# dmalyuta/explicit_hybrid_mpc

Hardware: AMD Instinct MI355X
Metric: oracle LP solves/sec + final regions/sec, 4-state 2-input N=5 hybrid MPC (higher is better)
Workload: dtype f64

## Files before the change

explicit_hybrid_mpc_amd/csrc/ehm_capi.hip:

```cpp
#include <hip/hip_runtime.h>

#include <algorithm>
#include <cmath>
#include <cstdarg>
#include <cstdio>
#include <cstdlib>
#include <cstring>
#include <functional>
#include <memory>
#include <set>
#include <string>
#include <vector>

#include "../../include/ehmpc.h"
#include "ehm_host.h"
#include "ehm_batch_host.h"

#define EHM_MAX_P_DEV 8
#include "ehm_kernels.h"
#include "ehm_k2.h"
#include "ehm_implicit.h"

using namespace ehm;

// ... 367 lines not shown
        const int id = nodes[t / (p + 1)];
        const int v = t % (p + 1);
        double* rec = T.rec + (size_t)id * T.rec_stride;
        if (lane < p) th[lane] = rec[v * p + lane];
        wave_sync();
        LpWork w;
        double b[EHM_SLOTS];
        assemble_point(w, lp_base, P, T.didx[id], th, false, b, lane);
        const IpmResult r = ipm_solve(w, b, lane);
        count_solve(cnt, r, lane);
        if (r.status != 0 && lane == 0) atomicAdd(&cnt->errors, 1ULL);
        if (lane == 0) rec[rec_off_vcost(p) + v] = r.obj;
        if (lane < n_u) rec[rec_off_vinput(p) + v * n_u + lane] = w.xb[lane];
    }
}

static thread_local ehm_err_channel g_err;

#define HIP_TRY(expr, code)                                                              \
    do {                                                                                 \
        hipError_t e_ = (expr);                                                          \
        if (e_ != hipSuccess)                                                            \
            return g_err.fail(code, "%s failed: %s (%s:%d)", #expr,                      \
                              hipGetErrorString(e_), __FILE__, __LINE__);                \
    } while (0)

struct NodePool {
    long long cap = 0;
    DevBuf rec, left, didx, depth, flags, tstar, grad, wit, mt_state, mt_data;
};

struct ehm_problem {
    int device = 0;
    Stream stream;
    DevProblem dp{};
    int delta_len = 0;
    std::vector<uint8_t> deltas;
    DevBuf consts;
    DevBuf wc2;
    DevBuf wc4;
    DevBuf wr3;
    DevBuf quad;
    bool quadratic = false;
    bool k2q_ok = false;
    bool v1_ok = false;
    int decide_full = 0;
    int mid_first = 1;
    int inherit_wit = 1;
    bool budget_keep = false;
    bool check_witness = false;
    int work_first = 1;
    int eager_children = 1;
    int requeue_undecided = 1;
    int share_mid = 1;
    int any_admissible = 0;
    int hy_timing = 0;
    int solver_gen = 2;
    DevBuf seg;
    std::set<const K2Api*> k2_ready;
    std::set<const KpApi*> kp_ready;
    NodePool pool_cache;
    DevBuf fr_a, fr_b, open_flag, open_list, d_count;
    DevBuf pq_slots, pq_ctl;
    DevBuf in0, in1, in2, out0, out1, out2, out3;
    DevBuf ex_stage, ex_tmp;
    DevBuf d_cnt;
    DevCounters* counters() const { return d_cnt.as<DevCounters>(); }
    struct ehm_tree* active_run = nullptr;
    std::vector<struct ehm_tree*> trees;
    Event bev[2];
    double batch_seconds[2] = {0.0, 0.0};
    long long batch_launches[2] = {0, 0};
    long long launches = 0;
    long long fallbacks = 0;
    long long slivers = 0;
    int num_cu = 256;
    size_t lds_point = 0, lds_simplex = 0, lds_expand = 0;
};

struct HyState;

struct ehm_tree {
    ehm_problem* prob = nullptr;
    int device = 0;
    std::unique_ptr<HyState> hy;
    DevTree dt{};
    NodePool pool;
    long long limit = 0;
    DevBuf code;
    ehm_tree_info info{};
    int skip_volume = 0;
    int32_t persist_kernel[4] = {0, 0, 0, 0};
    bool unordered = false;
    bool keep_ids = false;
    DevBuf d_perm, d_inv;
    bool have_perm = false;
    struct Run {
        bool active = false;
        int max_depth = 0, action = 0, shard_world = 1, shard_rank = 0, engine = 0;
        int deal_depth = 0;
        long long shard_min = 0;
        bool sharded = true, cur_is_a = true;
        long long n_roots = 0, n_nodes = 0, nf = 0, n_closed = 0, ref_solves = 0;
        long long pre_closed = 0, pre_nodes = 0, pre_solves = 0, given = 0, received = 0;
        long long pre_first = 0;
        long long pushes = 0;
        int sweeps = 0, depth = 0, truncated = 0;
        DevCounters c0{};
        Event ev0;
        std::vector<Event> evs;
        std::vector<int> ev_kind;
    } run;
    ~ehm_tree();
};

static int map_deltas(ehm_problem* P, int64_t n_inst, const uint8_t* delta,
                      std::vector<int32_t>& out) {
    out.resize((size_t)n_inst);
    const int L = P->delta_len;
    for (int64_t k = 0; k < n_inst; ++k) {
// ... 496 lines not shown
        return g_err.fail(EHM_E_NO_DEVICE, "no HIP device %d (libehmpc has no CPU fallback)",
                          device);
    HIP_TRY(hipSetDevice(device), EHM_E_NO_DEVICE);
    DevBuf d_out;
    HIP_TRY(d_out.alloc(5 * sizeof(double)), EHM_E_HIP);
    int k = 0;
    for (k2_getter g : g_k2_getters) {
        if (k >= max_instances) break;
        g()->selftest(nullptr, d_out.as<double>());
        HIP_TRY(hipDeviceSynchronize(), EHM_E_HIP);
        HIP_TRY(hipMemcpy(out + 5 * k, d_out.ptr, 5 * sizeof(double), hipMemcpyDeviceToHost),
                EHM_E_HIP);
        ++k;
    }
    *n_instances = k;
    return EHM_OK;
}

int ehm_problem_set_option(ehm_problem* P, const char* name, double value) {
    if (!P || !name) return g_err.fail(EHM_E_INVALID, "null argument");
    if (!strcmp(name, "solver")) return ehm_problem_set_solver(P, (int)value);
    if (!strcmp(name, "decide_full")) {
        P->decide_full = value != 0.0;
        return EHM_OK;
    }
    if (!strcmp(name, "timing")) {
        P->hy_timing = value != 0.0;
        return EHM_OK;
    }
    if (!strcmp(name, "mid_first")) {
        P->mid_first = value != 0.0;
        return EHM_OK;
    }
    if (!strcmp(name, "inherit_witness")) {
        P->inherit_wit = value != 0.0;
        return EHM_OK;
    }
    if (!strcmp(name, "work_first")) {
        P->work_first = value != 0.0;
        return EHM_OK;
    }
    if (!strcmp(name, "check_witness")) {
        P->check_witness = value != 0.0;
        return EHM_OK;
    }
    if (!strcmp(name, "eager_children")) {
        P->eager_children = value != 0.0;
        return EHM_OK;
    }
    if (!strcmp(name, "requeue_undecided")) {
        P->requeue_undecided = value != 0.0;
        return EHM_OK;
    }
    if (!strcmp(name, "budget_keep")) {
        P->budget_keep = value != 0.0;
        return EHM_OK;
    }
    if (!strcmp(name, "share_midpoints")) {
        P->share_mid = value != 0.0;
        return EHM_OK;
    }
    if (!strcmp(name, "any_admissible")) {
        if (value < 0.0 || value > 2e9)
            return g_err.fail(EHM_E_INVALID, "any_admissible: seed + 1, or 0");
        if (P->active_run)
            return g_err.fail(EHM_E_INVALID, "any_admissible: not while a partition run is active");
        P->any_admissible = (int)value;
        return EHM_OK;
    }
    return g_err.fail(EHM_E_INVALID, "unknown option '%s'", name);
}

int ehm_sync(ehm_problem* P) {
    if (!P) return g_err.fail(EHM_E_INVALID, "null problem");
    HIP_TRY(hipStreamSynchronize(P->stream), EHM_E_HIP);
    return EHM_OK;
}

void* ehm_stream(ehm_problem* P) { return P ? (void*)P->stream : nullptr; }

int ehm_stats(ehm_problem* P, ehm_counters* out) {
    if (!P || !out) return g_err.fail(EHM_E_INVALID, "null argument");
    HIP_TRY(hipSetDevice(P->device), EHM_E_HIP);
    DevCounters c;
    HIP_TRY(hipStreamSynchronize(P->stream), EHM_E_HIP);
    HIP_TRY(hipMemcpy(&c, P->counters(), sizeof c, hipMemcpyDeviceToHost), EHM_E_HIP);
    out->lp_solves = (int64_t)c.lp_solves;
    out->ipm_iters = (int64_t)c.ipm_iters;
    out->stalled = (int64_t)c.stalled;
    out->kernel_launches = P->launches;
    out->fallbacks = P->fallbacks;
    out->slivers = P->slivers;
    for (int k = 0; k < 2; ++k) {
        out->batch_seconds[k] = P->batch_seconds[k];
        out->batch_launches[k] = P->batch_launches[k];
    }
    return EHM_OK;
}

struct BatchIn {
    const double* host;
    size_t width;
    DevBuf* dev;
};
struct BatchOut {
    void* host;
// ... 1190 lines not shown
        }
    }
    const long long waves = (long long)cfg.L.grid * (cfg.L.threads / 64);
    const long long n_slots = 2 * T->limit + waves + 64;
    if (n_slots > 0x7fffffffLL || T->limit >= (long long)EHM_REQUEUED)
        return g_err.fail(EHM_E_INVALID, "node pool too large for the persistent engine");
    HIP_TRY(P->pq_slots.ensure((size_t)n_slots * 4), EHM_E_HIP);
    HIP_TRY(P->pq_ctl.ensure(sizeof(PersistCtl)), EHM_E_HIP);
    int32_t* slots = P->pq_slots.as<int32_t>();
    HIP_TRY(hipMemsetAsync(slots, 0xFF, (size_t)n_slots * 4, P->stream), EHM_E_HIP);
    const int32_t* cur = (R.cur_is_a ? P->fr_a : P->fr_b).as<int32_t>();
    HIP_TRY(hipMemcpyAsync(slots, cur, (size_t)R.nf * 4, hipMemcpyDeviceToDevice, P->stream),
            EHM_E_HIP);
    PersistDeal deal{0, 0, 0, 1, 0, 0, 0, 0};
    deal.check = P->check_witness ? 1 : 0;
    T->dt.code = nullptr;
    if (dealt) {
        deal = PersistDeal{0, R.deal_depth, R.shard_rank, R.shard_world,
                           getenv("EHM_DEAL_LOW_BITS") ? 0 : 1, 0, P->check_witness ? 1 : 0, 0};
        HIP_TRY(T->code.ensure((size_t)T->pool.cap * 4), EHM_E_HIP);
        T->dt.code = T->code.as<uint32_t>();
        std::vector<uint32_t> codes((size_t)R.n_roots);
        for (long long k = 0; k < R.n_roots; ++k) codes[(size_t)k] = (uint32_t)k;
        HIP_TRY(hipMemcpyAsync(T->dt.code, codes.data(), codes.size() * 4, hipMemcpyHostToDevice,
                               P->stream), EHM_E_HIP);
        HIP_TRY(hipStreamSynchronize(P->stream), EHM_E_HIP);
    }
    if (max_pops > 0 && max_pops < n_slots) deal.pop_limit = (int)max_pops;
    deal.keep = (P->work_first && !getenv("EHM_NO_WORKFIRST")) ? 1 : 0;
    if (deal.pop_limit > 0 && !P->budget_keep) deal.keep = 0;
    deal.eager = P->eager_children ? 1 : 0;
    deal.requeue = P->requeue_undecided ? 1 : 0;
    PersistCtl h{};
    h.head = 0;
    h.tail = (int)R.nf;
    h.pending = (int)R.nf;
    h.n_nodes = (int)R.n_nodes;
    HIP_TRY(hipMemcpyAsync(P->pq_ctl.ptr, &h, sizeof h, hipMemcpyHostToDevice, P->stream),
            EHM_E_HIP);
    R.evs.push_back(Event::recorded(P->stream));
    if (kp) {
        T->persist_kernel[0] = kp_mid ? EHM_PERSIST_KPM : EHM_PERSIST_KP;
        T->persist_kernel[1] = kp->np_decide;
        T->persist_kernel[2] = kp->np_expand;
        T->persist_kernel[3] = kp->slots;
    } else {
        T->persist_kernel[0] = cfg.api == ehm_k4_api() ? EHM_PERSIST_K4 : EHM_PERSIST_K2;
        T->persist_kernel[1] = cfg.api->np;
        T->persist_kernel[2] = cfg.api->np;
        T->persist_kernel[3] = cfg.api->slots;
    }
    (kp ? kp->persist : cfg.api->persist)(cfg.L, P->dp, T->dt, slots, (int)n_slots,
                                          P->pq_ctl.as<PersistCtl>(), (int)T->limit, P->counters(),
                                          P->decide_full ? 0 : 1, R.max_depth, deal);
    R.evs.push_back(Event::recorded(P->stream));
    R.ev_kind.push_back(0);
    P->launches++;
    HIP_TRY(hipGetLastError(), EHM_E_HIP);
    HIP_TRY(hipMemcpyAsync(&h, P->pq_ctl.ptr, sizeof h, hipMemcpyDeviceToHost, P->stream),
            EHM_E_HIP);
    HIP_TRY(hipStreamSynchronize(P->stream), EHM_E_HIP);
    if (h.abort == 1)
        return g_err.fail(EHM_E_CAPACITY, "node pool exhausted at %d nodes (max_nodes=%lld)",
                          h.n_nodes, T->limit);
    const long long left_over =
        (deal.pop_limit > 0 && h.tail > deal.pop_limit) ? (long long)h.tail - deal.pop_limit : 0;
    if (h.abort != 0 || h.pending != left_over)
        return g_err.fail(EHM_E_HIP,
                          "persistent frontier kernel stopped early (abort=%d, pending=%d, "
                          "expected %lld)", h.abort, h.pending, left_over);
    if (left_over > 0) {
        DevBuf& fb = P->fr_a;
        HIP_TRY(fb.ensure((size_t)left_over * 4 * 2), EHM_E_HIP);
        HIP_TRY(hipMemcpyAsync(fb.ptr, slots + deal.pop_limit, (size_t)left_over * 4,
                               hipMemcpyDeviceToDevice, P->stream), EHM_E_HIP);
        HIP_TRY(hipStreamSynchronize(P->stream), EHM_E_HIP);
        R.cur_is_a = true;
    }
    R.ref_solves += (long long)h.closed + 3LL * (long long)h.splits;
    R.pushes += (long long)h.pushes;
    if (deal.world > 1) {
        R.pre_closed = (long long)h.repl_closed;
        R.pre_nodes = R.n_roots + 2LL * (long long)h.repl_splits;
        R.pre_solves = (long long)h.repl_solves;
        R.sharded = true;
    }
    R.n_closed += (long long)h.closed;
    R.n_nodes = h.n_nodes;
    R.truncated = R.truncated || h.truncated;
    R.depth = std::max(R.depth, h.max_depth_seen);
    R.sweeps = R.depth + 1;
    R.nf = left_over;
    T->unordered = true;
    return EHM_OK;
}

int ehm_partition_advance(ehm_tree* T, int64_t max_pops, int64_t* frontier_size) {
    if (!T || !T->run.active) return g_err.fail(EHM_E_INVALID, "no partition run in progress");
    ehm_problem* P = T->prob;
    auto& R = T->run;
    if (T->hy || P->solver_gen != 2 || P->dp.Wr3)
        return g_err.fail(EHM_E_INVALID,
                          "ehm_partition_advance: needs a single-commutation problem on "
                          "the shared-block kernels (use ehm_partition_step)");
    HIP_TRY(hipSetDevice(P->device), EHM_E_HIP);
    int rc = EHM_OK;
    T->keep_ids = true;
// ... 30 lines not shown
                           EHM_OK &&
                       pc.api->persist != nullptr;
    }
    const bool want_persist = R.engine == 1 && P->solver_gen == 2 && max_sweeps <= 0 &&
                              (!P->dp.Wr3 || wide_persist);
    if (want_persist && R.nf > 0 && (R.shard_world == 1 || R.sharded || R.deal_depth > 0)) {
        int rc = persistent_run(T);
        if (frontier_size) *frontier_size = 0;
        return rc;
    }
    DevBuf &fr_a = P->fr_a, &fr_b = P->fr_b, &open_flag = P->open_flag,
           &open_list = P->open_list, &d_count = P->d_count;
    auto stamp = [&]() { R.evs.push_back(Event::recorded(P->stream)); };
    int done = 0;
    while (R.nf > 0 && !R.truncated && (max_sweeps <= 0 || done < max_sweeps)) {
        int32_t* cur = (R.cur_is_a ? fr_a : fr_b).as<int32_t>();
        if (!R.sharded && R.nf >= R.shard_min) {
            DevBuf& ob = R.cur_is_a ? fr_b : fr_a;
            HIP_TRY(ob.ensure((size_t)(R.nf / R.shard_world + 1) * 4), EHM_E_HIP);
            hipLaunchKernelGGL(k_shard_filter, dim3((unsigned)((R.nf + 255) / 256)), dim3(256), 0,
                               P->stream, T->dt, cur, (int)R.nf, R.shard_rank, R.shard_world,
                               ob.as<int32_t>());
            P->launches++;
            cur = ob.as<int32_t>();
            R.cur_is_a = !R.cur_is_a;
            R.pre_first = (R.sweeps == 0) ? 0 : R.n_nodes - R.nf;
            R.nf = (R.nf - R.shard_rank + R.shard_world - 1) / R.shard_world;
            R.sharded = true;
            DevCounters cs;
            int rc2 = read_counters(P, cs);
            if (rc2) return rc2;
            R.pre_closed = R.n_closed;
            R.pre_nodes = R.n_nodes;
            R.pre_solves = (long long)(cs.lp_solves - R.c0.lp_solves);
            if (R.nf == 0) break;
            if (want_persist) {
                int rc3 = persistent_run(T);
                if (frontier_size) *frontier_size = 0;
                return rc3;
            }
        }
        if ((long long)open_flag.cap < R.nf * 4) {
            HIP_TRY(open_flag.ensure((size_t)R.nf * 4 * 2), EHM_E_HIP);
            HIP_TRY(open_list.ensure((size_t)R.nf * 4 * 2), EHM_E_HIP);
        }
        K2Cfg cfg_d;
        if (P->solver_gen == 2) {
            int rc = k2_config(P, LP_SLACK, LP_SLACK, R.nf, cfg_d);
            if (rc) return rc;
        }
        stamp();
        if (P->solver_gen == 2)
            cfg_d.api->decide(cfg_d.L, P->dp, T->dt, cur, (int)R.nf, open_flag.as<int32_t>(),
                              P->counters(), P->decide_full ? 0 : 1);
        else
            hipLaunchKernelGGL(k_lcss_decide, dim3(grid_for(P, R.nf)), dim3(64), P->lds_simplex,
                               P->stream, P->dp, T->dt, cur, (int)R.nf, open_flag.as<int32_t>(),
                               P->counters());
        stamp();
        R.ev_kind.push_back(0);
        hipLaunchKernelGGL(k_scan_open, dim3(1), dim3(1024), 0, P->stream,
                           open_flag.as<int32_t>(), cur, (int)R.nf, open_list.as<int32_t>(),
                           d_count.as<int32_t>());
        P->launches += 2;
        int32_t n_open = 0;
        {
            hipError_t e = hipMemcpyAsync(&n_open, d_count.ptr, 4, hipMemcpyDeviceToHost,
                                          P->stream);
            if (e == hipSuccess) e = hipStreamSynchronize(P->stream);
            if (e != hipSuccess)
                return g_err.fail(EHM_E_HIP, "sweep %d failed: %s", R.sweeps, hipGetErrorString(e));
        }
        ++R.sweeps;
        ++done;
        R.ref_solves += R.nf;
        R.n_closed += R.nf - n_open;
        if (n_open == 0) {
            R.nf = 0;
            break;
        }
        if (R.max_depth > 0 && R.depth >= R.max_depth) {
            R.truncated = 1;
            break;
        }
        if (R.n_nodes + 2LL * n_open > T->limit)
            return g_err.fail(EHM_E_CAPACITY, "node pool exhausted at %lld nodes (max_nodes=%lld)",
                              R.n_nodes, T->limit);
        DevBuf& nb = R.cur_is_a ? fr_b : fr_a;
        if ((long long)nb.cap < 2LL * n_open * 4) {
            HIP_TRY(nb.ensure((size_t)n_open * 2 * 4 * 2), EHM_E_HIP);
        }
        int32_t* nxt = nb.as<int32_t>();
        K2Cfg cfg_e;
        if (P->solver_gen == 2) {
            int rc = k2_config(P, LP_POINT, LP_POINT, n_open, cfg_e);
            if (rc) return rc;
        }
        stamp();
        if (P->solver_gen == 2)
            cfg_e.api->expand(cfg_e.L, P->dp, T->dt, open_list.as<int32_t>(), (int)n_open,
                              (int)R.n_nodes, nxt, P->counters());
        else
            hipLaunchKernelGGL(k_lcss_expand, dim3(grid_for(P, n_open)), dim3(64), P->lds_expand,
                               P->stream, P->dp, T->dt, open_list.as<int32_t>(), (int)n_open,
                               (int)R.n_nodes, nxt, P->counters());
        stamp();
        R.ev_kind.push_back(1);
// ... 404 lines not shown
```

explicit_hybrid_mpc_amd/csrc/ehm_dev.h:

```cpp
#pragma once

#include <hip/hip_runtime.h>
#include <stdint.h>

namespace ehm {

struct DevProblem {
    int n, m, p, n_u, n_delta;
    const double* Gt;
    const double* St;
    const double* w;
    const double* c;
    double eps_a, eps_r;
    const double* Wc2;
    int lda2, ncw2;
    const double* Wc4;
    int lda4, ncw4, tot4;
    int nd0, LE4;
    int wc_lds;
    const double* Wr3;
    int mpad3;
    const double* Hq;
    const double* Fq;
    const double* f0q;
    const double* Cq;
    const double* c1q;
    const double* c0q;
};

}
#include "ehm_midtable.h"
namespace ehm {

struct DevTree {
    double*  rec;
    int32_t* left;
    int32_t* didx;
    int32_t* depth;
    uint8_t* flags;
    double*  tstar;
    int rec_stride;
    int p, n_u;
    double*  grad;
    uint32_t* code;
    double*  wit;
    MidTable mt;
};

#define EHM_WIT_REL 0.02

__device__ __forceinline__ void witness_for_children(const double* wit, const double* Vc, int bi,
                                                     int bj, int lane, double& v0, double& v1) {
    const double ai = wit[1 + bi], aj = wit[1 + bj];
    const bool to0 = aj >= ai;
    const double an = to0 ? aj : ai, af = to0 ? ai : aj;
    const int far = to0 ? bi : bj;
    const int near = to0 ? bj : bi;
    const double mu = (an - af) / (1.0 + an - af);
    double vh = wit[lane], vo = (1.0 - mu) * wit[lane];
    if (lane == 0) vo = fma(mu, Vc[far], vo);
    if (lane == 1 + far) {
        vh = 2.0 * af;
        vo = 0.0;
    }
    if (lane == 1 + near) {
        vh = an - af;
        vo = 2.0 * (1.0 - mu) * an;
    }
    v0 = to0 ? vh : vo;
    v1 = to0 ? vo : vh;
}

__device__ inline double cut_bound(const double* node, const double* g, int p, double eps_a,
                                   double eps_r, int lane, double* scr, double thr = -1e301) {
    const int na = p + 1, nr = 2 * na;
    const double* V = node + na * p;
    for (int k = lane; k < na * na; k += 64) {
        const int i = k / na, j = k - i * na;
        double d = 0.0;
        for (int q = 0; q < p; ++q) d = fma(g[i * p + q], node[j * p + q] - node[i * p + q], d);
        const double Li = V[i] + d;
        scr[(2 * i) * na + j] = V[j] - Li - eps_a;
        scr[(2 * i + 1) * na + j] = V[j] - (1.0 + eps_r) * Li;
    }
    __builtin_amdgcn_fence(__ATOMIC_ACQ_REL, "wavefront");
    __builtin_amdgcn_wave_barrier();
    double b = 1e300;
    if (lane < nr) {
        double m = -1e300;
        bool ok = true;
        for (int j = 0; j < na; ++j) {
            const double f = scr[lane * na + j];
            ok = ok && (f == f);
            m = fmax(m, f);
        }
        if (ok) b = m;
    }
    if (thr > -1e300) {
        double b1 = b;
#pragma unroll
        for (int o = 8; o > 0; o >>= 1) b1 = fmin(b1, __shfl_xor(b1, o, 64));
        const double b1a = __shfl(b1, 0, 64), b1b = __shfl(b1, 16, 64);
        b1 = fmin(b1a, b1b);
// ... 159 lines not shown
```

explicit_hybrid_mpc_amd/csrc/ehm_ipm2.h:

```cpp
#include "ehm_dev.h"

#ifndef EHM_NP
#error "EHM_NP (column capacity, multiple of 4) must be defined"
#endif
#ifndef EHM_SLOTS
#error "EHM_SLOTS (row slots per lane) must be defined"
#endif

#ifndef EHM2_UNROLL
#define EHM2_UNROLL 2
#endif
#ifndef EHM2_FORM_MFMA
#define EHM2_FORM_MFMA 0
#endif
#ifndef EHM2_LU_CHUNK
#define EHM2_LU_CHUNK 8
#endif
#define EHM2_TOL_RES      1e-10
#define EHM2_TOL_GAP      1e-10
#define EHM2_MAX_ITER     40
#define EHM2_STEP_FRAC    0.999
#define EHM2_STEP_FRAC_SAFE 0.99
#define EHM2_STEP_FRAC_LAST 0.9
#define EHM2_ATTEMPTS     3
// ... 1317 lines not shown
                few_sums(rs2, W.nE);
                rho0 = rs2[0];
                rho1 = rs2[1];
            } else {
                rho0 = few_sum(l2 ? xr[0] * q : 0.0, W.nE);
            }
        }
    }
    double l = 0.0, i1 = 0.0, i2 = 0.0;
    if (kd > 0) {
        l = W.dn[0];
        i1 = W.dn[1];
        i2 = W.dn[2];
        rho1 = fma(-l, rho0, rho1);
        rr = fma(-W.xh[jl], i1 * rho0, rr);
        rr = fma(-W.xh[NP + jl], i2 * rho1, rr);
    }
    const double xD = lu_solve(row, W, rinv, rr, lane);
    double y0 = 0.0, y1 = 0.0;
    if (kd > 0 && W.nE > 0) {
        const bool lr = lane < W.nr;
        double v0, v1 = 0.0;
        if (two) {
            double vs[2] = {lr ? W.xh[jl] * xD : 0.0, lr ? W.xh[NP + jl] * xD : 0.0};
            few_sums(vs, W.nr);
            v0 = vs[0] + rho0;
            v1 = vs[1] + rho1;
        } else {
            v0 = few_sum(lr ? W.xh[jl] * xD : 0.0, W.nr) + rho0;
        }
        y1 = v1 * i2;
        y0 = fma(-l, y1, v0 * i1);
    }
    if (W.nE > 0) {
        double xE = 0.0;
        if (el) {
            double acc = rhs;
            const double* ge = W.gE + e * GS;
            for (int j = 0; j < W.nr; ++j) acc = fma(-ge[j], W.t[j], acc);
            if (kd > 0) {
                const double* xr = W.X + (size_t)(W.nr + e) * W.ldx;
                acc = fma(-xr[0], y0, acc);
                if (two) acc = fma(-xr[1], y1, acc);
            }
            xE = acc * W.iD[e];
            W.t[W.nr + e] = xE;
        }
        wsync();
        return el ? xE : xD;
    }
    return xD;
}

__device__ __forceinline__ IpmResult ipm_solve(const Shared& S, const Wave& W, const double (&b)[SLOTS],
                                      int lane0, int sign_only, double step_frac,
                                      double* gout = nullptr) {
    int lane = lane0;
    const int n = W.n_lp;
    const int m_lp = S.m + W.ne;
    RowMap rm;
    make_rowmap(rm, S, W, lane);
    double s[SLOTS], lam[SLOTS], v[SLOTS];
    double bmax = 0.0;
#pragma unroll
    for (int sl = 0; sl < SLOTS; ++sl) {
        v[sl] = rm.valid[sl] ? b[sl] : 0.0;
        s[sl] = rm.valid[sl] ? fmax(b[sl], 1.0) : 1.0;
        lam[sl] = rm.valid[sl] ? 1.0 : 0.0;
        bmax = fmax(bmax, fabs(v[sl]));
    }
    const double bnorm = uniform_d(1.0 + wave_max_nn(bmax));
    const double cj = (lane < n) ? W.c[lane] : 0.0;
    const double cnorm = uniform_d(1.0 + wave_max_nn(fabs(cj)));
    step_frac = uniform_d(step_frac);
    if (lane < n) {
        W.x[lane] = 0.0;
        W.xb[lane] = 0.0;
    }
#pragma unroll
    for (int sl = 0; sl < SLOTS; ++sl) {
        if (!rm.valid[sl]) {
            W.vm0[lane + 64 * sl] = 0.0;
            W.vm1[lane + 64 * sl] = 0.0;
        }
    }
    wsync();

#if EHM2_PROF
    if (lane0 < 24) W.pf[lane0] = 0ULL;
    wsync();
    long long _tp = (long long)__builtin_readcyclecounter();
#endif
    IpmResult res;
    res.obj = 0.0;
    res.merit = const_d(1e300);
    res.iters = 0;
    res.status = 1;
    int stall = 0;
    int m_op = __builtin_amdgcn_readfirstlane(m_lp);
    asm volatile("" : "+s"(m_op));
    const double inv_m = uniform_d(frcp((double)m_op));

    for (int it = 0; it <= EHM2_MAX_ITER; ++it) {
        lane = pin(lane0);
#if EHM2_QUAD
        double xQx = 0.0, qx = 0.0, gjj = 0.0;
// ... 16 lines not shown
                    W.X[(size_t)lane * W.ldx + W.eq - W.nsx] = fma(W.kap1, gvj, a1j);
                    W.X[(size_t)lane * W.ldx + W.eq - W.nsx + 1] = fma(W.kap2, gvj, a2j);
                }
                const double a1x = wave_sum(a1j * xj);
                const double a2x = wave_sum(a2j * xj);
                const int e = lane + 64 * (SLOTS - 1) - W.xbase;
                const double Vx = fma(0.5, xQx, qx);
                if (rm.last_extra && e == W.eq) v[SLOTS - 1] = W.bq1 - fma(W.kap1, Vx, a1x);
                if (rm.last_extra && e == W.eq + 1) v[SLOTS - 1] = W.bq2 - fma(W.kap2, Vx, a2x);
            }
            wsync();
        }
#endif
        double r_p[SLOTS], rs[SLOTS];
        double rpmax = 0.0, sl_sum = 0.0, vl_sum = 0.0;
#pragma unroll
        for (int sl = 0; sl < SLOTS; ++sl) {
            r_p[sl] = rm.valid[sl] ? (s[sl] - v[sl]) : 0.0;
            rpmax = fmax(rpmax, fabs(r_p[sl]));
            sl_sum = fma(s[sl], lam[sl], sl_sum);
            vl_sum = fma(v[sl], lam[sl], vl_sum);
            rs[sl] = frcp(s[sl]);
        }
#pragma unroll
        for (int sl = 0; sl < SLOTS; ++sl) {
            if (rm.valid[sl]) {
                W.vm0[lane + 64 * sl] = lam[sl];
                W.vm1[lane + 64 * sl] = lam[sl] * rs[sl] * r_p[sl];
            }
        }
        wsync();
        EHM2_PT(0)
        double atl, atdr;
        cols_times<true>(S, W, W.vm0, W.vm1, W.M, lane, atl, atdr);
        EHM2_PT(1)
        const double cjj = (lane < n) ? W.c[lane] : 0.0;
        const double xjj = (lane < n) ? W.x[lane] : 0.0;
#if EHM2_QUAD
        const double r_d = (lane < n) ? (atl + cjj + gjj) *
            (W.quad ? rsqrt(1.0 + W.Q[lane * LDM + lane]) : 1.0) : 0.0;
        const double cn = W.quad ? (1.0 + wave_max_nn(fmax(fabs(cjj), fabs(gjj)))) : cnorm;
        const double emax = wave_max_nn(fmax(rpmax / bnorm, fabs(r_d) / cn));
        const double sl_tot = wave_sum(sl_sum);
        const double mu = sl_tot * inv_m;
        double pobj = wave_sum(cjj * xjj);
        double dobj = -wave_sum(vl_sum + xjj * atl);
        if (W.quad) {
            pobj += W.kap0 * (fma(0.5, xQx, qx) + W.v0);
            dobj = pobj - sl_tot;
        }
        const double e_g = fabs(pobj - dobj) / (1.0 + fabs(pobj));
#else
        const double r_d = (lane < n) ? (atl + cjj) : 0.0;
        const double emax = wave_max_nn(fmax(rpmax / bnorm, fabs(r_d) / cnorm));
        double sums[3] = {sl_sum, vl_sum + xjj * atl, cjj * xjj};
        wave_sums(sums);
        const double mu = sums[0] * inv_m;
        const double dobj = -sums[1];
        const double pobj = sums[2];
        const double e_g = fabs(pobj - dobj) / (1.0 + fabs(pobj));
#endif
        const double merit = fmax(emax / const_d(EHM2_TOL_RES), e_g / const_d(EHM2_TOL_GAP));
        if (!(mu == mu) || !(pobj == pobj) || fabs(pobj) > const_d(1e300)) {
            res.merit = const_d(1e300);
            res.obj = pobj;
            res.status = 1;
            res.iters = it;
            break;
        }
        if (merit < res.merit) {
            res.merit = uniform_d(merit);
            res.obj = uniform_d(pobj);
            stall = 0;
            if (lane < n) W.xb[lane] = W.x[lane];
        } else if (res.merit < const_d(EHM2_STALL_ZONE)) {
            ++stall;
        }
        res.iters = it;
        if (merit <= 1.0) {
            res.status = 0;
            break;
        }
        if (sign_only && emax <= const_d(EHM2_SIGN_RES) && pobj * dobj > 0.0 &&
            (sign_only == 1 || pobj > 0.0)) {
            const double lo = fmin(fabs(pobj), fabs(dobj));
            if (lo >= W.sign_floor && fabs(pobj - dobj) <= const_d(EHM2_SIGN_GAP) * lo &&
                emax * (1.0 + fabs(pobj)) <= const_d(EHM2_SIGN_RES_REL) * lo) {
                res.obj = pobj;
                res.merit = merit;
                res.margin = lo;
                res.status = 0;
                if (lane < n) W.xb[lane] = W.x[lane];
                wsync();
                EHM2_PT(15)
                EHM2_PDUMP()
                return res;
            }
        }
        if (stall >= 3 || it == EHM2_MAX_ITER || !(merit == merit)) break;

        EHM2_PT(15)
        lane = pin(lane0);
#pragma unroll
        for (int sl = 0; sl < SLOTS; ++sl)
            if (rm.valid[sl]) W.vm0[lane + 64 * sl] = lam[sl] * rs[sl];
        wsync();
        if (rm.last_extra || rm.last_sx >= 0)
            W.ub[lane + 64 * (SLOTS - 1) - W.xbase] = lam[SLOTS - 1] * rs[SLOTS - 1];
#if EHM2_QUAD
        if (W.quad && W.eq >= 0 && rm.last_extra) {
            const int e = lane + 64 * (SLOTS - 1) - W.xbase;
            if (e == W.eq) W.lq[0] = lam[SLOTS - 1];
            if (e == W.eq + 1) W.lq[1] = lam[SLOTS - 1];
        }
#endif
        wsync();
#if EHM2_PROF
        form_normal_matrix(S, W, W.vm0, W.ub, lane, lane0, _tp);
#else
        form_normal_matrix(S, W, W.vm0, W.ub, lane);
#endif
        EHM2_PT(4)
        lane = pin(lane0);
        dense_prep(S, W, W.ub, lane);
        EHM2_PT(5)
        lane = pin(lane0);
        double row[NP];
        {
            const int jr = (lane < NP) ? lane : (NP - 1);
            const double* mrow = W.M + jr * LDM;
#pragma unroll
            for (int q = 0; q < NP; ++q) row[q] = mrow[q];
            double dg = mrow[jr];
            for (int r = 0; r < W.ne - W.nsx; ++r) {
                const double* xh = W.xh + r * NP;
                const double xl = xh[jr];
                const double ce = W.dn[1 + r] * xl;
                dg = fma(ce, xl, dg);
#pragma unroll
                for (int q = 0; q < NP; ++q) {
                    row[q] = fma(ce, xh[q], row[q]);
                    if ((q & 3) == 3) __builtin_amdgcn_sched_barrier(0);
                }
            }
#if EHM2_QUAD
            if (W.quad) {
                double wq = W.kap0;
                if (W.eq >= 0) wq = fma(W.kap1, W.lq[0], fma(W.kap2, W.lq[1], wq));
                const int jl = (lane < NP) ? lane : (NP - 1);
                const double* qrow = W.Q + jl * LDM;
                const bool in = jl < W.n_lp;
// ... 129 lines not shown
```

explicit_hybrid_mpc_amd/csrc/ehm_k2.hip:

```cpp
#include <hip/hip_runtime.h>

#include "ehm_k2_asm.h"

using namespace ehm;

namespace EHM2_NS {

#if EHM2_PROF
#define K2_PROF_HOOK(S) S.gprof = cnt ? cnt->phase : nullptr;
#else
#define K2_PROF_HOOK(S)
#endif
#define K2_PROLOGUE()                                                            \
    double* sm = reinterpret_cast<double*>(k2_smem);                             \
    __shared__ int s_ctr;                                                        \
    const int tid = threadIdx.x;                                                 \
    const int lane0 = tid & 63;                                                  \
    const int wave = __builtin_amdgcn_readfirstlane(tid >> 6);    \
    Shared S;                                                                    \
    carve_shared(S, sm, P);                                                      \
    K2_PROF_HOOK(S)                                                              \
    NodeBuf nb;                                                                  \
    carve_node(nb, sm + shared_doubles(P) + (size_t)wave * wave_doubles, P.p, P.n_u)

// ... 172 lines not shown
                if (lane == 0) alpha[o * (p + 1)] = 1.0 - sb;
            }
            wsync();
        }
        pos = run_end;
    }
}

__global__ __launch_bounds__(EHM_K2_THREADS) void k2_lcss_decide(
    DevProblem P, DevTree T, const int32_t* __restrict__ frontier, int nf,
    int32_t* __restrict__ open_flag, DevCounters* cnt, int wave_doubles, int sign_only) {
    K2_PROLOGUE();
    const int nrec = rec_doubles(P.p, P.n_u);
    const int per = (nf + gridDim.x - 1) / gridDim.x;
    const int lo = blockIdx.x * per;
    const int hi = (lo + per < nf) ? lo + per : nf;
    if (lo >= hi) return;
    load_shared(P, 0, sm, tid, blockDim.x);
    if (tid == 0) s_ctr = lo;
    __syncthreads();
    for (;;) {
        const int f = pull(&s_ctr, lane0);
        if (f >= hi) break;
        const int lane = pin(lane0);
        const int id = frontier[f];
        const double* rec = T.rec + (size_t)id * T.rec_stride;
        for (int k = lane; k < nrec; k += 64) nb.rec[k] = rec[k];
        wsync();
        if (T.grad && sign_only) {
            const double thr = -EHM_ROUTE_TOL * (1.0 + fabs(nb.rec[rec_off_vcost(P.p)]));
            const double bnd = cut_bound(nb.rec, T.grad + (size_t)id * (P.p + 1) * P.p, P.p,
                                         P.eps_a, P.eps_r, lane, nb.lp, thr);
            if (bnd < thr) {
                if (lane == 0) {
                    atomicAdd(&cnt->cert_closed, 1ULL);
                    T.tstar[id] = bnd;
                    open_flag[f] = 0;
                    T.flags[id] |= 1;
                    atomicMin(&cnt->min_margin_bits,
                              (unsigned long long)__double_as_longlong(-bnd));
                }
                wsync();
                continue;
            }
        }
        Wave W;
        IpmResult r;
        int its = 0;
        for (int attempt = 0; attempt < EHM2_ATTEMPTS; ++attempt) {
            double b[SLOTS];
            const int ln = pin(lane);
            assemble_simplex(S, W, nb, nb.rec, nb.rec + rec_off_vcost(P.p), SX_SLACK, P.eps_a,
                             P.eps_r, b, ln, P, 0);
            r = ipm_solve(S, W, b, ln, sign_only != 0,
                          step_fraction(attempt));
            its += r.iters;
            if (r.status == 0) break;
        }
        r.iters = its;
        count_solve(cnt, r, lane);
        if (lane == 0) {
            if (r.status != 0) {
                atomicAdd(&cnt->errors, 1ULL);
                T.flags[id] |= 8;
            }
            atomicAdd(&cnt->slack_solves, 1ULL);
            atomicAdd(&cnt->slack_iters, (unsigned long long)r.iters);
            const double t = -r.obj;
            const bool open = (t >= 0.0);
            T.tstar[id] = t;
            open_flag[f] = open ? 1 : 0;
            if (!open) T.flags[id] |= 1;
            atomicMin(&cnt->min_margin_bits, (unsigned long long)__double_as_longlong(r.margin));
            if (r.margin < EHM_ROUTE_TOL * (1.0 + fabs(nb.rec[rec_off_vcost(P.p)])))
                atomicAdd(&cnt->routed, 1ULL);
        }
        wsync();
    }
}

__global__ __launch_bounds__(EHM_K2_THREADS) void k2_lcss_expand(
    DevProblem P, DevTree T, const int32_t* __restrict__ open_list, int n_open, int child_base,
    int32_t* __restrict__ next_frontier, DevCounters* cnt, int wave_doubles) {
    K2_PROLOGUE();
    const int p = P.p, n_u = P.n_u;
    const int nrec = rec_doubles(p, n_u);
    const int per = (n_open + gridDim.x - 1) / gridDim.x;
    const int lo = blockIdx.x * per;
    const int hi = (lo + per < n_open) ? lo + per : n_open;
    if (lo >= hi) return;
    load_shared(P, 0, sm, tid, blockDim.x);
    if (tid == 0) s_ctr = lo;
    __syncthreads();
    for (;;) {
        const int f = pull(&s_ctr, lane0);
        if (f >= hi) break;
        const int lane = pin(lane0);
        const int id = open_list[f];
        const double* rec = T.rec + (size_t)id * T.rec_stride;
        double* node = nb.rec;
        double* mid = nb.th;
        for (int k = lane; k < nrec; k += 64) node[k] = rec[k];
        wsync();
        int bi, bj;
        longest_edge_wave(node, p, lane, bi, bj);
        if (lane < p) {
#pragma clang fp contract(off)
            mid[lane] = (node[bi * p + lane] + node[bj * p + lane]) / 2.0;
// ... 230 lines not shown
```

explicit_hybrid_mpc_amd/csrc/ehm_persist.h:

```cpp
#ifndef EHM_PERSIST_H
#define EHM_PERSIST_H

#ifndef kx_persist
#error "kx_persist (the kernel's name) must be defined, and the namespace aliases kd / ke declared"
#endif

#define EHM_PERSIST_WATCHDOG_TICKS (60LL * 100000000LL)
#ifndef EHM_PERSIST_MIDFIRST
#define EHM_PERSIST_MIDFIRST 0
#endif
__global__ __launch_bounds__(EHM_K2_THREADS) void kx_persist(
    DevProblem P, DevTree T, int32_t* slots, int n_slots, PersistCtl* ctl, int node_cap,
    DevCounters* cnt, int wave_doubles, int sign_only, int max_depth, PersistDeal deal) {
    double* sm = reinterpret_cast<double*>(k2_smem);
    const int tid = threadIdx.x;
    const int lane0 = tid & 63;
    const int wave = __builtin_amdgcn_readfirstlane(tid >> 6);
    kd::Shared S;
    kd::carve_shared(S, sm, P);
    ke::Shared Se;
    ke::carve_shared(Se, sm, P);
#if EHM2_PROF
    S.gprof = cnt ? cnt->phase : nullptr;
    Se.gprof = cnt ? cnt->phase : nullptr;
// ... 321 lines not shown
                        for (int k = 0; k < p; ++k) em[k] = (node[ea * p + k] + node[eb * p + k]) / 2.0;
                    }
                    unsigned int e_i = 0u;
                    const unsigned long long e_tg = mt_tag(em, p, T.mt.mask, &e_i);
                    slot_l = mt_find(T.mt, e_tg, e_i);
                }
            }
            if (__builtin_amdgcn_ballot_w64(slot_l >= 0) != 0ull) {
                __builtin_amdgcn_fence(__ATOMIC_ACQUIRE, "agent");
                if (slot_l >= 0) {
                    const double* e = T.mt.data + (size_t)slot_l * MT_DOUBLES;
                    bool same = true;
                    for (int k = 0; k < p; ++k)
                        same = same && __double_as_longlong(e[k]) == __double_as_longlong(em[k]);
                    const int word = (int)e[9];
                    if (same && (word & 0xff) == 0 && ((word >> 8) & 1)) {
                        J_l = e[8];
                        const double vb = 0.5 * (Vc[ea] + Vc[eb]);
                        const double tw = fmin(vb - J_l - P.eps_a, vb - (1.0 + P.eps_r) * J_l);
                        if (tw > EHM_ROUTE_TOL * (1.0 + fabs(vb))) tw_l = tw;
                    }
                }
                const unsigned long long won = __builtin_amdgcn_ballot_w64(tw_l > -1e299);
                if (won != 0ull) {
                    const int src = __builtin_ctzll(won);
                    const double tw = __shfl(tw_l, src);
                    const double Jw = __shfl(J_l, src);
                    const int wa = __shfl(ea, src), wb = __shfl(eb, src);
                    open = true;
                    decided = true;
                    tst = tw;
                    margin = tw;
                    if (T.wit) {
                        if (lane == 0) wit[0] = Jw;
                        if (lane <= p) wit[1 + lane] = (lane == wa || lane == wb) ? 0.5 : 0.0;
                        have_wit = true;
                    }
                    if (lane == 0) wst[W_WITT] += 1;
                    kd::wsync();
                }
            }
        }
#endif
        if (!decided) {
            const long long t_slk = wall_clock64();
            kd::Wave W;
            kd::IpmResult r;
            its = 0;
            for (int attempt = 0; attempt < EHM2_ATTEMPTS; ++attempt) {
                double b[kd::SLOTS];
                const int ln = kd::pin(lane);
                kd::assemble_simplex(S, W, nb, node, node + rec_off_vcost(p), SX_SLACK, P.eps_a,
                                     P.eps_r, b, ln, P, 0);
                r = kd::ipm_solve(S, W, b, ln, sign_only != 0, kd::step_fraction(attempt));
                its += r.iters;
                if (r.status == 0) break;
            }
            tst = -r.obj;
            open = (tst >= 0.0);
            margin = r.margin;
            const int slack_status = r.status;
#if !EHM2_QUAD
            if (T.wit && sign_only && open && slack_status == 0) {
                const int nz = S.n;
                double cz = 0.0, sb = 0.0;
                for (int q = 0; q < nz; ++q) cz = fma(S.cv[q], W.xb[kd::zcol(W, S, q)], cz);
                for (int q = 0; q < p; ++q) sb += W.xb[W.psi0 + q];
                kd::wsync();
                if (lane == 0) {
                    wit[0] = fma(EHM_WIT_REL, margin, cz);
                    wit[1] = 1.0 - sb;
                }
                if (lane < p) wit[2 + lane] = W.xb[W.psi0 + lane];
                have_wit = true;
                kd::wsync();
            }
#endif
            if (lane == 0) {
                wst[W_TSLK] += (unsigned long long)(wall_clock64() - t_slk);
                wst[W_SOLVES] += 1;
                if (dep < deal.depth) wst[W_RSOLVES] += 1;
                wst[W_ITERS] += (unsigned long long)its;
                wst[W_SLACK] += 1;
                wst[W_SLACK_ITERS] += (unsigned long long)its;
                if (slack_status != 0) {
                    wst[W_STALLED] += 1;
                    wst[W_ERRORS] += 1;
                    T.flags[id] |= 8;
                }
            }
        }
        if (lane == 0) {
            if (can_split) {
                if (mt_res != MT_HIT) {
                    wst[W_SOLVES] += 1;
                    if (dep < deal.depth) wst[W_RSOLVES] += 1;
                    wst[W_ITERS] += (unsigned long long)mid_iters;
                }
                if (mid_status != 0 && open) {
                    wst[W_STALLED] += 1;
                    wst[W_ERRORS] += 1;
                    T.flags[id] |= 16;
                }
            }
            *wmargin = fmin(*wmargin, margin);
            if (margin < EHM_ROUTE_TOL * (1.0 + fabs(node[rec_off_vcost(p)]))) wst[W_ROUTED] += 1;
            if ((unsigned long long)dep > wst[W_DEPTH]) wst[W_DEPTH] = (unsigned long long)dep;
// ... 28 lines not shown
        const double gv0 = (T.grad && lane < ng) ? T.grad[(size_t)id * ng + lane] : 0.0;
        const int d = is_hot ? hot_d : T.didx[id];
        int c0 = c0_early;
        if (!alloc_early && lane == 0) c0 = atomicAdd(&ctl->n_nodes, 2);
        c0 = __builtin_amdgcn_readfirstlane(c0);
        if (c0 + 2 > node_cap) {
            if (lane == 0) {
                atomicMax(&ctl->abort, 1);
                atomicSub(&ctl->pending, 1);
            }
            break;
        }
        struct { double obj; } r = {Jm};
        if (T.grad) {
            const double* gp_ = T.grad + (size_t)id * ng;
            double* g0 = T.grad + (size_t)c0 * ng;
            for (int k = lane; k < ng; k += 64) {
                const double gv = (k < 64) ? gv0 : gp_[k];
                const double a0 = (k >= bi * p && k < bi * p + p) ? stash[st_g + k - bi * p] : gv;
                const double a1 = (k >= bj * p && k < bj * p + p) ? stash[st_g + k - bj * p] : gv;
                __hip_atomic_store(g0 + k, a0, __ATOMIC_RELAXED, __HIP_MEMORY_SCOPE_AGENT);
                __hip_atomic_store(g0 + ng + k, a1, __ATOMIC_RELAXED, __HIP_MEMORY_SCOPE_AGENT);
                if (stage) hgrad[k] = a1;
                if (eager) hg0[k] = a0;
            }
        }
        if (T.wit && lane < p + 2) {
            double* w0 = T.wit + (size_t)c0 * (p + 2);
            double v0 = 0.0, v1 = 0.0;
            if (have_wit) {
                witness_for_children(wit, node + rec_off_vcost(p), bi, bj, lane, v0, v1);
            }
            __hip_atomic_store(w0 + lane, v0, __ATOMIC_RELAXED, __HIP_MEMORY_SCOPE_AGENT);
            __hip_atomic_store(w0 + (p + 2) + lane, v1, __ATOMIC_RELAXED, __HIP_MEMORY_SCOPE_AGENT);
            kd::wsync();
            if (stage) wit[lane] = v1;
            if (eager) cw0[lane] = v0;
        }
        if (lane == 0) {
            wst[W_SPLITS] += 1;
            if (dep < deal.depth) wst[W_RSPLITS] += 1;
        }
        const double* xmid = stash;
#else
        kd::IpmResult r;
        int its = 0;
        {
            kd::Wave W;
            for (int attempt = 0; attempt < EHM2_ATTEMPTS; ++attempt) {
                double b[kd::SLOTS];
                const int ln = kd::pin(lane);
                kd::assemble_simplex(S, W, nb, node, node + rec_off_vcost(p), SX_SLACK, P.eps_a,
                                     P.eps_r, b, ln, P, 0);
                r = kd::ipm_solve(S, W, b, ln, sign_only != 0, kd::step_fraction(attempt));
                its += r.iters;
                if (r.status == 0) break;
            }
        }
        r.iters = its;
        const double tst = -r.obj;
        const bool open = (tst >= 0.0);
        if (lane == 0) {
            wst[W_SOLVES] += 1;
            if (dep < deal.depth) wst[W_RSOLVES] += 1;
            wst[W_ITERS] += (unsigned long long)r.iters;
            wst[W_SLACK] += 1;
            wst[W_SLACK_ITERS] += (unsigned long long)r.iters;
            if (r.status != 0) {
                wst[W_STALLED] += 1;
                wst[W_ERRORS] += 1;
                T.flags[id] |= 8;
            }
            *wmargin = fmin(*wmargin, r.margin);
            if (r.margin < EHM_ROUTE_TOL * (1.0 + fabs(node[rec_off_vcost(p)]))) wst[W_ROUTED] += 1;
            if ((unsigned long long)dep > wst[W_DEPTH]) wst[W_DEPTH] = (unsigned long long)dep;
            T.tstar[id] = tst;
            if (!open) {
                T.flags[id] |= 1;
                wst[W_CLOSED] += 1;
                if (dep < deal.depth) wst[W_RCLOSED] += 1;
            }
        }
        if (!open) {
            if (lane == 0) atomicSub(&ctl->pending, 1);
            kd::wsync();
            continue;
        }
        if (max_depth > 0 && dep >= max_depth) {
            if (lane == 0) {
                wst[W_TRUNC] = 1;
                atomicSub(&ctl->pending, 1);
            }
            kd::wsync();
            continue;
        }
        int c0 = 0;
        if (lane == 0) c0 = atomicAdd(&ctl->n_nodes, 2);
        c0 = __builtin_amdgcn_readfirstlane(c0);
        if (c0 + 2 > node_cap) {
            if (lane == 0) {
                atomicMax(&ctl->abort, 1);
                atomicSub(&ctl->pending, 1);
            }
            break;
        }
        double* mid = nb.th;
        int bi, bj;
// ... 215 lines not shown
```

Measured before the change: 11.18 million.

## Stop slack-LP IPM early once one side's objective bound certifies the sign

Adds a one-sided early-termination test to the interior-point solver used in decide and persistent kernels. Primal and dual residuals are now reduced separately. The solve returns as soon as the dual objective is positive with small dual residual, or optionally (mode 2) the primal objective is negative with small primal residual, so there is no need to wait for both sides and the gap to converge. This cuts IPM iterations per node, at the cost of an extra wave reduction per iteration and a looser certificate that relies on weak duality holding at the stopping iterate. The option defaults on.

After: 11.18 million. About the same (-0.0%).

```diff
diff --git a/explicit_hybrid_mpc_amd/csrc/ehm_capi.hip b/explicit_hybrid_mpc_amd/csrc/ehm_capi.hip
--- a/explicit_hybrid_mpc_amd/csrc/ehm_capi.hip
+++ b/explicit_hybrid_mpc_amd/csrc/ehm_capi.hip
@@ -443,6 +443,7 @@
     int work_first = 1;
     int eager_children = 1;
     int requeue_undecided = 1;
+    int one_sided_stop = 1;
     int share_mid = 1;
     int any_admissible = 0;
     int hy_timing = 0;
@@ -457,6 +458,10 @@
     DevBuf ex_stage, ex_tmp;
     DevBuf d_cnt;
     DevCounters* counters() const { return d_cnt.as<DevCounters>(); }
+    int decide_sign_bits() const {
+        return decide_full ? 0 : (1 | (one_sided_stop ? EHM_SIGN_ONE_SIDED : 0) |
+                                   (one_sided_stop == 2 ? EHM_SIGN_PRIMAL_SIDE : 0));
+    }
     struct ehm_tree* active_run = nullptr;
     std::vector<struct ehm_tree*> trees;
     Event bev[2];
@@ -1059,6 +1064,12 @@
         P->requeue_undecided = value != 0.0;
         return EHM_OK;
     }
+    if (!strcmp(name, "one_sided_stop")) {
+        if (value != 0.0 && value != 1.0 && value != 2.0)
+            return g_err.fail(EHM_E_INVALID, "one_sided_stop: 0, 1 or 2");
+        P->one_sided_stop = (int)value;
+        return EHM_OK;
+    }
     if (!strcmp(name, "budget_keep")) {
         P->budget_keep = value != 0.0;
         return EHM_OK;
@@ -2355,7 +2366,7 @@
     }
     (kp ? kp->persist : cfg.api->persist)(cfg.L, P->dp, T->dt, slots, (int)n_slots,
                                           P->pq_ctl.as<PersistCtl>(), (int)T->limit, P->counters(),
-                                          P->decide_full ? 0 : 1, R.max_depth, deal);
+                                          P->decide_sign_bits(), R.max_depth, deal);
     R.evs.push_back(Event::recorded(P->stream));
     R.ev_kind.push_back(0);
     P->launches++;
@@ -2492,7 +2503,7 @@
         stamp();
         if (P->solver_gen == 2)
             cfg_d.api->decide(cfg_d.L, P->dp, T->dt, cur, (int)R.nf, open_flag.as<int32_t>(),
-                              P->counters(), P->decide_full ? 0 : 1);
+                              P->counters(), P->decide_sign_bits());
         else
             hipLaunchKernelGGL(k_lcss_decide, dim3(grid_for(P, R.nf)), dim3(64), P->lds_simplex,
                                P->stream, P->dp, T->dt, cur, (int)R.nf, open_flag.as<int32_t>(),
diff --git a/explicit_hybrid_mpc_amd/csrc/ehm_dev.h b/explicit_hybrid_mpc_amd/csrc/ehm_dev.h
--- a/explicit_hybrid_mpc_amd/csrc/ehm_dev.h
+++ b/explicit_hybrid_mpc_amd/csrc/ehm_dev.h
@@ -49,6 +49,9 @@
 
 #define EHM_WIT_REL 0.02
 
+#define EHM_SIGN_ONE_SIDED 4
+#define EHM_SIGN_PRIMAL_SIDE 8
+
 __device__ __forceinline__ void witness_for_children(const double* wit, const double* Vc, int bi,
                                                      int bj, int lane, double& v0, double& v1) {
     const double ai = wit[1 + bi], aj = wit[1 + bj];
diff --git a/explicit_hybrid_mpc_amd/csrc/ehm_ipm2.h b/explicit_hybrid_mpc_amd/csrc/ehm_ipm2.h
--- a/explicit_hybrid_mpc_amd/csrc/ehm_ipm2.h
+++ b/explicit_hybrid_mpc_amd/csrc/ehm_ipm2.h
@@ -1393,6 +1393,7 @@
     return xD;
 }
 
+template <bool ONE_SIDED = false>
 __device__ __forceinline__ IpmResult ipm_solve(const Shared& S, const Wave& W, const double (&b)[SLOTS],
                                       int lane0, int sign_only, double step_frac,
                                       double* gout = nullptr) {
@@ -1515,7 +1516,14 @@
         const double e_g = fabs(pobj - dobj) / (1.0 + fabs(pobj));
 #else
         const double r_d = (lane < n) ? (atl + cjj) : 0.0;
-        const double emax = wave_max_nn(fmax(rpmax / bnorm, fabs(r_d) / cnorm));
+        double eres[2] = {rpmax / bnorm, fabs(r_d) / cnorm};
+        if (ONE_SIDED) {
+            wave_maxs_nn(eres);
+        } else {
+            eres[0] = eres[1] = wave_max_nn(fmax(eres[0], eres[1]));
+        }
+        const double e_p = eres[0], e_d = eres[1];
+        const double emax = fmax(e_p, e_d);
         double sums[3] = {sl_sum, vl_sum + xjj * atl, cjj * xjj};
         wave_sums(sums);
         const double mu = sums[0] * inv_m;
@@ -1544,8 +1552,9 @@
             res.status = 0;
             break;
         }
-        if (sign_only && emax <= const_d(EHM2_SIGN_RES) && pobj * dobj > 0.0 &&
-            (sign_only == 1 || pobj > 0.0)) {
+        const int sign_mode = sign_only & 3;
+        if (sign_mode && emax <= const_d(EHM2_SIGN_RES) && pobj * dobj > 0.0 &&
+            (sign_mode == 1 || pobj > 0.0)) {
             const double lo = fmin(fabs(pobj), fabs(dobj));
             if (lo >= W.sign_floor && fabs(pobj - dobj) <= const_d(EHM2_SIGN_GAP) * lo &&
                 emax * (1.0 + fabs(pobj)) <= const_d(EHM2_SIGN_RES_REL) * lo) {
@@ -1560,6 +1569,27 @@
                 return res;
             }
         }
+#if !EHM2_QUAD
+        if (ONE_SIDED && (sign_only & 3) == 1 && (sign_only & EHM_SIGN_ONE_SIDED)) {
+            const bool dual = dobj > W.sign_floor && e_d <= const_d(EHM2_SIGN_RES) &&
+                e_d * (1.0 + fabs(dobj)) <= const_d(EHM2_SIGN_RES_REL) * dobj;
+            const bool prim = (sign_only & EHM_SIGN_PRIMAL_SIDE) && pobj < -W.sign_floor &&
+                e_p <= const_d(EHM2_SIGN_RES) &&
+                e_p * (1.0 + fabs(pobj)) <= const_d(EHM2_SIGN_RES_REL) * fabs(pobj);
+            if (prim || dual) {
+                const double bound = prim ? pobj : dobj;
+                res.obj = bound;
+                res.merit = merit;
+                res.margin = fabs(bound);
+                res.status = 0;
+                if (lane < n) W.xb[lane] = W.x[lane];
+                wsync();
+                EHM2_PT(15)
+                EHM2_PDUMP()
+                return res;
+            }
+        }
+#endif
         if (stall >= 3 || it == EHM2_MAX_ITER || !(merit == merit)) break;
 
         EHM2_PT(15)
diff --git a/explicit_hybrid_mpc_amd/csrc/ehm_k2.hip b/explicit_hybrid_mpc_amd/csrc/ehm_k2.hip
--- a/explicit_hybrid_mpc_amd/csrc/ehm_k2.hip
+++ b/explicit_hybrid_mpc_amd/csrc/ehm_k2.hip
@@ -248,8 +248,7 @@
             const int ln = pin(lane);
             assemble_simplex(S, W, nb, nb.rec, nb.rec + rec_off_vcost(P.p), SX_SLACK, P.eps_a,
                              P.eps_r, b, ln, P, 0);
-            r = ipm_solve(S, W, b, ln, sign_only != 0,
-                          step_fraction(attempt));
+            r = ipm_solve<true>(S, W, b, ln, sign_only, step_fraction(attempt));
             its += r.iters;
             if (r.status == 0) break;
         }
diff --git a/explicit_hybrid_mpc_amd/csrc/ehm_persist.h b/explicit_hybrid_mpc_amd/csrc/ehm_persist.h
--- a/explicit_hybrid_mpc_amd/csrc/ehm_persist.h
+++ b/explicit_hybrid_mpc_amd/csrc/ehm_persist.h
@@ -397,7 +397,7 @@
                 const int ln = kd::pin(lane);
                 kd::assemble_simplex(S, W, nb, node, node + rec_off_vcost(p), SX_SLACK, P.eps_a,
                                      P.eps_r, b, ln, P, 0);
-                r = kd::ipm_solve(S, W, b, ln, sign_only != 0, kd::step_fraction(attempt));
+                r = kd::ipm_solve<true>(S, W, b, ln, sign_only, kd::step_fraction(attempt));
                 its += r.iters;
                 if (r.status == 0) break;
             }
@@ -532,7 +532,7 @@
                 const int ln = kd::pin(lane);
                 kd::assemble_simplex(S, W, nb, node, node + rec_off_vcost(p), SX_SLACK, P.eps_a,
                                      P.eps_r, b, ln, P, 0);
-                r = kd::ipm_solve(S, W, b, ln, sign_only != 0, kd::step_fraction(attempt));
+                r = kd::ipm_solve<true>(S, W, b, ln, sign_only, kd::step_fraction(attempt));
                 its += r.iters;
                 if (r.status == 0) break;
             }
```
